# sharinka0715/semantic-gaussians

Hardware: NVIDIA H100
Metric: Mviews/s + HBM GB/s, 1M Gaussians, 256-ch features, 1080p, fwd+bwd (higher is better)
Workload: dtype f32

## Files before the change

semantic-gaussians_b200/csrc/chn_dfeature.cu:

```cuda
#include <cstddef>
#include <cstring>
#include "chn_blend.cuh"
#include "tma.cuh"

namespace sgb {

namespace {

constexpr int kDfCH = 256;
constexpr int kDfStages = 4;
constexpr int kDfPass = 128;
constexpr int kDfSlabPix = 32;
constexpr int kDfSlabs = SGB_TILE_PIX / kDfSlabPix;
constexpr int kDfComputeWarps = kDfCH / 32;
constexpr int kDfThreads = 128 + 32 * kDfComputeWarps;
constexpr uint32_t kDfProducerRegs = 56, kDfComputeRegs = 224;
static_assert(128 * kDfProducerRegs + 32 * kDfComputeWarps * kDfComputeRegs <= 65536,
              "dL/dfeature: the warp groups' register limits exceed the register file");

struct DfHdr {
    int end;
    int cnt;
    int slab;
    int ch0, nch;
    uint32_t gid[kDfPass];
};
template <typename T>
struct DfSmem {
    float w[kDfStages][kDfPass * kDfSlabPix];
    T dl[kDfStages][kDfSlabPix * kDfCH];
    DfHdr hdr[kDfStages];
    uint64_t full[kDfStages], empty[kDfStages];
};
template <typename T>
constexpr size_t kDfSmemBytes = sizeof(DfSmem<T>) + 1024;
static_assert(kDfSmemBytes<float> <= 227 * 1024, "dL/dfeature shared memory exceeds the sm_90 opt-in limit");

__device__ __forceinline__ void df_setmaxnreg_dec() {
    asm volatile("setmaxnreg.dec.sync.aligned.u32 %0;" ::"n"(kDfProducerRegs));
}
__device__ __forceinline__ void df_setmaxnreg_inc() {
    asm volatile("setmaxnreg.inc.sync.aligned.u32 %0;" ::"n"(kDfComputeRegs));
}

template <typename T>
__device__ __forceinline__ int df_swz(int cl) { return sizeof(T) == 4 ? (cl >> 1) & 3 : (cl >> 2) & 1; }
__device__ __forceinline__ float4 df_dl4(const float* dl, int q, int k, int swz, int rs) {
    return *reinterpret_cast<const float4*>(dl + (q >> 2) * rs + k * 16 + (((q & 3) ^ swz ^ (k >> 1)) << 2));
}
__device__ __forceinline__ float4 df_dl4(const __half* dl, int q, int k, int swz, int rs) {
    const uint2 r = *reinterpret_cast<const uint2*>(dl + (q >> 2) * rs + k * 16 + ((((q & 3) >> 1) ^ swz) << 3) +
                                                    ((q & 1) << 2));
    const float2 a = __half22float2(*reinterpret_cast<const __half2*>(&r.x));
    const float2 b = __half22float2(*reinterpret_cast<const __half2*>(&r.y));
    return make_float4(a.x, a.y, b.x, b.y);
}

__device__ __forceinline__ void cp_async4(void* dst_smem, const void* src, int src_bytes) {
    asm volatile("cp.async.ca.shared.global [%0], [%1], 4, %2;" ::"r"(smem_u32(dst_smem)), "l"(src), "r"(src_bytes)
                 : "memory");
}
__device__ __forceinline__ void cp_async_mbar_arrive_noinc(uint64_t* bar) {
    asm volatile("cp.async.mbarrier.arrive.noinc.shared::cta.b64 [%0];" ::"r"(smem_u32(bar)) : "memory");
}

template <int R, typename T>
__device__ __forceinline__ void df_slab(float (&acc)[8][16], const float* __restrict__ ws, const T* __restrict__ dl,
                                        int rs, int eg, int swz) {
#pragma unroll 1
    for (int q = 0; q < kDfSlabPix / 4; q++) {
        float4 d[16];
#pragma unroll
        for (int k = 0; k < 16; k++) d[k] = df_dl4(dl + (k >> 2) * (8 * 16), q, k & 3, swz, rs);
#pragma unroll
        for (int j = 0; j < R; j++) {
            const float4 wv = *reinterpret_cast<const float4*>(ws + (eg + 16 * j) * 32 + ((q ^ (eg & 7)) << 2));
#pragma unroll
            for (int k = 0; k < 16; k++) {
                acc[j][k] = fmaf(wv.x, d[k].x, acc[j][k]);
                acc[j][k] = fmaf(wv.y, d[k].y, acc[j][k]);
                acc[j][k] = fmaf(wv.z, d[k].z, acc[j][k]);
                acc[j][k] = fmaf(wv.w, d[k].w, acc[j][k]);
            }
        }
    }
}

template <typename T>
__global__ void __launch_bounds__(kDfThreads, 1) dfeature_persistent_kernel(
    int W, int H, int C, int CW, const T* __restrict__ dL_dpixels, PoolView pool, float* __restrict__ dL_dcolors,
    int* __restrict__ work_counter, const __grid_constant__ CUtensorMap dl_map,
    const __grid_constant__ CUtensorMap w_map, const int use_tma) {
    extern __shared__ __align__(128) unsigned char smem_raw[];
    DfSmem<T>& sm = *reinterpret_cast<DfSmem<T>*>(smem_raw + ((1024u - (smem_u32(smem_raw) & 1023u)) & 1023u));
    const int tid = threadIdx.x, lane = tid & 31, warp = tid >> 5;
    if (tid == 0) {
        for (int i = 0; i < kDfStages; i++) {
            mbar_init(&sm.full[i], use_tma ? 1 : 33);
            mbar_init(&sm.empty[i], kDfComputeWarps);
        }
        mbar_fence_init();
    }
    __syncthreads();

    if (warp >= 4) {
        df_setmaxnreg_inc();
        const int cw = warp - 4;
        const int eg = lane >> 1;
        const int cl = cw * 32 + (lane & 1) * 4;
        const int rs = CW * 16;
        const int swz = df_swz<T>(cl);
        const bool red16 = ((C & 3) == 0) && ((reinterpret_cast<uintptr_t>(dL_dcolors) & 15) == 0);
        float acc[8][16];
        for (uint32_t step = 0;; step++) {
            const int st = (int)(step % kDfStages);
            mbar_wait(&sm.full[st], (step / kDfStages) & 1u);
            const DfHdr& h = sm.hdr[st];
            if (h.end) break;
            const int slab = h.slab, cnt = h.cnt, nch = h.nch;
            const int R = (cnt + 15) >> 4;
            if (slab == 0) {
#pragma unroll
                for (int j = 0; j < 8; j++)
#pragma unroll
                    for (int k = 0; k < 16; k++) acc[j][k] = 0.f;
            }
            if (cw * 32 < nch) {
                const float* ws = sm.w[st];
                const T* dl = sm.dl[st] + cl * 16;
                switch (R) {
                    case 1: df_slab<1, T>(acc, ws, dl, rs, eg, swz); break;
                    case 2: df_slab<2, T>(acc, ws, dl, rs, eg, swz); break;
                    case 3: df_slab<3, T>(acc, ws, dl, rs, eg, swz); break;
                    case 4: df_slab<4, T>(acc, ws, dl, rs, eg, swz); break;
                    case 5: df_slab<5, T>(acc, ws, dl, rs, eg, swz); break;
                    case 6: df_slab<6, T>(acc, ws, dl, rs, eg, swz); break;
                    case 7: df_slab<7, T>(acc, ws, dl, rs, eg, swz); break;
                    default: df_slab<8, T>(acc, ws, dl, rs, eg, swz); break;
                }
                if (slab == kDfSlabs - 1) {
                    const int ch0 = h.ch0;
#pragma unroll
                    for (int j = 0; j < 8; j++) {
                        const int e = eg + 16 * j;
                        if (j >= R || e >= cnt) continue;
                        float* dst = dL_dcolors + (size_t)h.gid[e] * C + ch0 + cl;
#pragma unroll
                        for (int g = 0; g < 4; g++) {
                            const int c = cl + 8 * g;
                            if (red16 && c + 4 <= nch) {
                                red_add_v4_f32(dst + 8 * g, make_float4(acc[j][4 * g], acc[j][4 * g + 1],
                                                                        acc[j][4 * g + 2], acc[j][4 * g + 3]));
                            } else {
#pragma unroll
                                for (int k = 0; k < 4; k++)
                                    if (c + k < nch) red_add_f32(dst + 8 * g + k, acc[j][4 * g + k]);
                            }
                        }
                    }
                }
            }
            __syncwarp();
            if (lane == 0) mbar_arrive(&sm.empty[st]);
        }
        return;
    }

    df_setmaxnreg_dec();
    if (warp != 0) return;
    const int tiles_x = (W + SGB_TILE - 1) / SGB_TILE;
    const int tiles = tiles_x * ((H + SGB_TILE - 1) / SGB_TILE);
    const int nitems = (C + CW - 1) / CW;
    const int total = tiles * nitems;
    const size_t plane = (size_t)H * W;
    const uint32_t dl_bytes = use_tma ? (uint32_t)(kDfSlabPix * CW * sizeof(T)) : 0u;
    uint32_t step = 0;
    auto acquire = [&]() -> int {
        const int st = (int)(step % kDfStages);
        if (step >= kDfStages) mbar_wait(&sm.empty[st], ((step / kDfStages) - 1) & 1u);
        return st;
    };
    for (;;) {
        int k = 0;
        if (lane == 0) k = atomicAdd(work_counter, 1);
        k = __shfl_sync(0xffffffffu, k, 0);
        if (k >= total) break;
        const int tile = k / nitems, ch0 = (k % nitems) * CW;
        const uint32_t n = pool.count[tile];
        if (n == 0) continue;
        const uint32_t dbase = pool.dirbase[tile];
        const int nch = min(CW, C - ch0);
        const int x0 = (tile % tiles_x) * SGB_TILE, y0 = (tile / tiles_x) * SGB_TILE;
        for (uint32_t base = 0; base < n; base += kDfPass) {
            const int cnt = (int)min((uint32_t)kDfPass, n - base);
            const int nck = (cnt + kChunkEntries - 1) / kChunkEntries;
            const uint32_t cid = lane < nck ? chunk_of(pool, dbase, (int)(base / kChunkEntries) + lane) : 0u;
            uint32_t gid[kDfPass / 32];
#pragma unroll
            for (int i = 0; i < kDfPass / 32; i++) {
                const int e = lane + 32 * i;
                const uint32_t c = __shfl_sync(0xffffffffu, cid, e / kChunkEntries);
                gid[i] = e < cnt ? pool.chunks[c].meta[e & (kChunkEntries - 1)].x : 0u;
            }
            for (int s = 0; s < kDfSlabs; s++) {
                const int st = acquire();
                DfHdr& h = sm.hdr[st];
                if (lane == 0) {
                    h.end = 0;
                    h.cnt = cnt;
                    h.slab = s;
                    h.ch0 = ch0;
                    h.nch = nch;
                }
                if (s == kDfSlabs - 1) {
#pragma unroll
                    for (int i = 0; i < kDfPass / 32; i++) h.gid[lane + 32 * i] = gid[i];
// ... 118 lines not shown
```

semantic-gaussians_b200/csrc/chn_forward.cu:

```cuda
#include "chn_blend.cuh"
#include "tma.cuh"

namespace sgb {

namespace {

template <int MCH>
__device__ __forceinline__ bool acc_nonfinite(const float2 (&acc)[8][MCH / 2]) {
    float2 z = make_float2(0.f, 0.f);
#pragma unroll
    for (int i = 0; i < 8; i++)
#pragma unroll
        for (int k = 0; k < MCH / 2; k++) z = ffma2(acc[i][k], make_float2(0.f, 0.f), z);
    const float t = z.x + z.y;
    return __any_sync(0xffffffffu, t != t);
}

template <int MCH, bool RING>
__device__ __noinline__ void forward_redo_guarded(const PoolView& pool, uint32_t n, uint32_t dbase,
                                                  const float* __restrict__ features, int C, int ch0, int nch,
                                                  int warp, int woff, int cg, const float* __restrict__ bg_color,
                                                  const float* __restrict__ final_T, int W, int H, uint32_t row,
                                                  uint32_t col0, float* __restrict__ out_color) {
    float acc[8][MCH];
#pragma unroll
    for (int i = 0; i < 8; i++)
#pragma unroll
        for (int k = 0; k < MCH; k++) acc[i][k] = 0.f;
    for (uint32_t e = 0; e < n; e++) {
        const WChunk* ck = pool.chunks + chunk_of(pool, dbase, (int)(e / kChunkEntries));
        const int s = (int)(e & (kChunkEntries - 1));
        const uint2 meta = ck->meta[s];
        if (!((meta.y >> warp) & 1u)) continue;
        const float* fr = features + (size_t)meta.x * C + ch0;
        float f[MCH];
#pragma unroll
        for (int k = 0; k < MCH; k++) {
            const int chl = RING ? ((k >> 2) * 32 + cg * 4 + (k & 3)) : (cg * MCH + k);
            f[k] = chl < nch ? __ldg(fr + chl) : 0.f;
        }
#pragma unroll
        for (int i = 0; i < 8; i++) {
            const float w = ck->w[s][woff + i];
            if (w != 0.f) {
#pragma unroll
                for (int k = 0; k < MCH; k++) acc[i][k] = fmaf(f[k], w, acc[i][k]);
            }
        }
    }
    if (row >= (uint32_t)H) return;
    const size_t plane = (size_t)H * W;
#pragma unroll
    for (int k = 0; k < MCH; k++) {
        const int chl = RING ? ((k >> 2) * 32 + cg * 4 + (k & 3)) : (cg * MCH + k);
        if (chl >= nch) continue;
        const float bgc = bg_color[ch0 + chl];
        float* dst = out_color + (size_t)(ch0 + chl) * plane + (size_t)W * row + col0;
#pragma unroll
        for (int i = 0; i < 8; i++)
            if (col0 + i < (uint32_t)W) dst[i] = acc[i][k] + final_T[(size_t)W * row + col0 + i] * bgc;
    }
}

template <int CH>
__global__ void __launch_bounds__(kTileThreads, 2) blend_forward_ldg_kernel(
    int W, int H, int C, const float* __restrict__ features, const float* __restrict__ bg_color,
    const float* __restrict__ final_T, PoolView pool, float* __restrict__ out_color) {
    constexpr int MCH = CH / 8;
    const int tiles_x = (W + SGB_TILE - 1) / SGB_TILE;
    const int nchunksC = (C + CH - 1) / CH;
    const int tile = blockIdx.x / nchunksC;
    const int ch0 = (blockIdx.x % nchunksC) * CH;
    const int nch = min(CH, C - ch0);
    const int tid = threadIdx.x, lane = tid & 31, warp = tid >> 5;
    const int pg = lane >> 3, cg = lane & 7;
    const uint2 pix_min = {(uint32_t)(tile % tiles_x) * SGB_TILE, (uint32_t)(tile / tiles_x) * SGB_TILE};

    float2 acc[8][MCH / 2];
#pragma unroll
    for (int i = 0; i < 8; i++)
#pragma unroll
        for (int k = 0; k < MCH / 2; k++) acc[i][k] = make_float2(0.f, 0.f);

    const uint32_t n = pool.count[tile];
    const uint32_t dbase = pool.dirbase[tile];
    const int woff = warp * 32 + pg * 8;
    const int foff = ch0 + cg * MCH;
    for (uint32_t e = 0; e < n;) {
        const WChunk* ck = pool.chunks + chunk_of(pool, dbase, (int)(e / kChunkEntries));
        const int m = (int)min((uint32_t)kChunkEntries, n - e);
        for (int s = 0; s < m; s++) {
            const uint2 meta = ck->meta[s];
            if (!((meta.y >> warp) & 1u)) continue;
            const float4* wp = reinterpret_cast<const float4*>(&ck->w[s][woff]);
            const float4 w0 = wp[0], w1 = wp[1];
            const float* fr = features + (size_t)meta.x * C + foff;
            float2 f[MCH / 2];
#pragma unroll
            for (int k = 0; k < MCH / 2; k++) {
                f[k].x = (cg * MCH + 2 * k < nch) ? __ldg(fr + 2 * k) : 0.f;
                f[k].y = (cg * MCH + 2 * k + 1 < nch) ? __ldg(fr + 2 * k + 1) : 0.f;
            }
            const float wv[8] = {w0.x, w0.y, w0.z, w0.w, w1.x, w1.y, w1.z, w1.w};
#pragma unroll
            for (int i = 0; i < 8; i++) {
                const float2 w2 = make_float2(wv[i], wv[i]);
#pragma unroll
                for (int k = 0; k < MCH / 2; k++) acc[i][k] = ffma2(f[k], w2, acc[i][k]);
            }
        }
        e += m;
    }
    const uint32_t row = pix_min.y + 2 * warp + (pg >> 1);
    const uint32_t col0 = pix_min.x + (pg & 1) * 8;
    if (acc_nonfinite<MCH>(acc)) {
        forward_redo_guarded<MCH, false>(pool, n, dbase, features, C, ch0, nch, warp, woff, cg, bg_color, final_T, W, H,
                                         row, col0, out_color);
        return;
    }
    if (row < (uint32_t)H) {
        const size_t plane = (size_t)H * W;
        const bool vec = ((W & 3) == 0) && (col0 + 8 <= (uint32_t)W);
        float Tv[8];
#pragma unroll
        for (int i = 0; i < 8; i++) Tv[i] = (col0 + i < (uint32_t)W) ? final_T[(size_t)W * row + col0 + i] : 0.f;
#pragma unroll
        for (int k = 0; k < MCH; k++) {
            const int chl = cg * MCH + k;
            if (chl >= nch) continue;
            const float bgc = bg_color[ch0 + chl];
            float* dst = out_color + (size_t)(ch0 + chl) * plane + (size_t)W * row + col0;
            float o[8];
#pragma unroll
            for (int i = 0; i < 8; i++) o[i] = ((k & 1) ? acc[i][k / 2].y : acc[i][k / 2].x) + Tv[i] * bgc;
            if (vec) {
                reinterpret_cast<float4*>(dst)[0] = make_float4(o[0], o[1], o[2], o[3]);
                reinterpret_cast<float4*>(dst)[1] = make_float4(o[4], o[5], o[6], o[7]);
            } else {
#pragma unroll
                for (int i = 0; i < 8; i++)
                    if (col0 + i < (uint32_t)W) dst[i] = o[i];
            }
        }
    }
}

template <int CH, int NS>
__global__ void __launch_bounds__(kTileThreads, 2) blend_forward_tma_kernel(
    int W, int H, int C, const float* __restrict__ features, const float* __restrict__ bg_color,
    const float* __restrict__ final_T, PoolView pool, float* __restrict__ out_color) {
    constexpr int MCH = CH / 8;
    constexpr int ES = kChunkEntries;
    constexpr int LA = NS - 2;
    constexpr int kDirCap = 192;
    struct Stage {
        float w[ES][SGB_TILE_PIX];
        float f[ES][CH];
    };
    extern __shared__ __align__(128) unsigned char smem_raw[];
    Stage* stg = reinterpret_cast<Stage*>(smem_raw);
    __shared__ uint64_t full_bar[NS], empty_bar[NS];
    __shared__ uint32_t Cdir[kDirCap];
    __shared__ __align__(16) float Tsm[SGB_TILE_PIX];
    __shared__ float bgS[CH];

    const int tiles_x = (W + SGB_TILE - 1) / SGB_TILE;
    const int nchunksC = (C + CH - 1) / CH;
    const int tile = blockIdx.x / nchunksC;
    const int ch0 = (blockIdx.x % nchunksC) * CH;
    const int nch = min(CH, C - ch0);
    const int tid = threadIdx.x, lane = tid & 31, warp = tid >> 5;
    const int pg = lane_group4(lane), cg = lane_group8(lane);
    const uint2 pix_min = {(uint32_t)(tile % tiles_x) * SGB_TILE, (uint32_t)(tile / tiles_x) * SGB_TILE};

    const uint32_t n = pool.count[tile];
    const int nb = (int)((n + ES - 1) / ES);
    const uint32_t dbase = pool.dirbase[tile];
    if (tid == 0) {
        for (int i = 0; i < NS; i++) {
            mbar_init(&full_bar[i], 1);
            mbar_init(&empty_bar[i], kTileThreads / 32);
        }
        mbar_fence_init();
    }
    for (int k = tid; k < min(nb, kDirCap); k += kTileThreads) Cdir[k] = chunk_of(pool, dbase, k);
    {
        const uint32_t x = pix_min.x + (tid & (SGB_TILE - 1)), y = pix_min.y + (tid >> 4);
        Tsm[tid] = (x < (uint32_t)W && y < (uint32_t)H) ? final_T[(size_t)W * y + x] : 0.f;
        if (tid < nch) bgS[tid] = bg_color[ch0 + tid];
    }
    if (nch < CH)
        for (int e = tid; e < NS * ES * CH; e += kTileThreads) {
            const int k = e % CH;
            if (k >= nch) stg[e / (ES * CH)].f[(e / CH) % ES][k] = 0.f;
        }
    __syncthreads();

    auto chunk_ptr = [&](int bi) {
        return pool.chunks + (bi < kDirCap ? Cdir[bi] : chunk_of(pool, dbase, bi));
    };
    auto load_meta = [&](int bi) {
        uint2 m = make_uint2(0u, 0u);
        if (bi < nb && lane < min(ES, (int)n - bi * ES)) m = __ldg(&chunk_ptr(bi)->meta[lane]);
        return m;
    };
    auto issue = [&](int bi, uint2 meta) {
        const int st = bi % NS;
        const int cnt = min(ES, (int)n - bi * ES);
        if (bi >= NS) mbar_wait(&empty_bar[st], (uint32_t)(((bi / NS) - 1) & 1));
        if (lane < cnt) {
            const WChunk* ck = chunk_ptr(bi);
            bulk_g2s(&stg[st].w[lane][0], &ck->w[lane][0], SGB_TILE_PIX * 4u, &full_bar[st]);
            bulk_g2s(&stg[st].f[lane][0], features + (size_t)meta.x * C + ch0, (uint32_t)nch * 4u, &full_bar[st]);
        }
        __syncwarp();
        if (lane == 0) mbar_arrive_expect_tx(&full_bar[st], (uint32_t)cnt * (SGB_TILE_PIX * 4u + (uint32_t)nch * 4u));
    };
    uint2 meta_next = make_uint2(0u, 0u);
    int pb = 0;
    if (warp == 0) {
        uint2 m[LA];
#pragma unroll
        for (int i = 0; i < LA; i++) m[i] = load_meta(i);
#pragma unroll
        for (int i = 0; i < LA; i++)
            if (i < nb) issue(i, m[i]);
        pb = min(LA, nb);
        meta_next = load_meta(pb);
    }

    float2 acc[8][MCH / 2];
#pragma unroll
    for (int i = 0; i < 8; i++)
#pragma unroll
        for (int k = 0; k < MCH / 2; k++) acc[i][k] = make_float2(0.f, 0.f);

    const int woff = warp * 32 + pg * 8;
    auto entry = [&](const Stage& sg, int e) {
        const float4 w0 = *reinterpret_cast<const float4*>(&sg.w[e][woff]);
        const float4 w1 = *reinterpret_cast<const float4*>(&sg.w[e][woff + 4]);
        float2 f[MCH / 2];
#pragma unroll
        for (int q = 0; q < MCH / 4; q++) {
            const float4 t = *reinterpret_cast<const float4*>(&sg.f[e][q * 32 + cg * 4]);
            f[2 * q] = make_float2(t.x, t.y);
            f[2 * q + 1] = make_float2(t.z, t.w);
        }
        const float wv[8] = {w0.x, w0.y, w0.z, w0.w, w1.x, w1.y, w1.z, w1.w};
#pragma unroll
        for (int i = 0; i < 8; i++) {
            const float2 w2 = make_float2(wv[i], wv[i]);
#pragma unroll
            for (int k = 0; k < MCH / 2; k++) acc[i][k] = ffma2(f[k], w2, acc[i][k]);
        }
    };
    for (int b = 0; b < nb; b++) {
        const int st = b % NS;
        const int cnt = min(ES, (int)n - b * ES);
        if (warp == 0 && pb < nb) {
            issue(pb, meta_next);
            pb++;
            meta_next = load_meta(pb);
        }
        mbar_wait(&full_bar[st], (uint32_t)((b / NS) & 1));
        if (cnt == ES) {
#pragma unroll
            for (int e = 0; e < ES; e++) entry(stg[st], e);
        } else {
            for (int e = 0; e < cnt; e++) entry(stg[st], e);
        }
        __syncwarp();
        if (lane == 0) mbar_arrive(&empty_bar[st]);
    }
    const uint32_t row = pix_min.y + 2 * warp + (pg >> 1);
    const uint32_t col0 = pix_min.x + (pg & 1) * 8;
    if (acc_nonfinite<MCH>(acc)) {
        forward_redo_guarded<MCH, true>(pool, n, dbase, features, C, ch0, nch, warp, woff, cg, bg_color, final_T, W, H,
                                        row, col0, out_color);
        return;
    }
    if (row < (uint32_t)H) {
        const size_t plane = (size_t)H * W;
        const bool vec = ((W & 3) == 0) && (col0 + 8 <= (uint32_t)W);
        const float4 t0 = *reinterpret_cast<const float4*>(&Tsm[(2 * warp + (pg >> 1)) * SGB_TILE + (pg & 1) * 8]);
        const float4 t1 = *reinterpret_cast<const float4*>(&Tsm[(2 * warp + (pg >> 1)) * SGB_TILE + (pg & 1) * 8 + 4]);
        const float Tv[8] = {t0.x, t0.y, t0.z, t0.w, t1.x, t1.y, t1.z, t1.w};
#pragma unroll
        for (int k = 0; k < MCH; k++) {
            const int chl = (k >> 2) * 32 + cg * 4 + (k & 3);
            if (chl >= nch) continue;
            const float bgc = bgS[chl];
            float* dst = out_color + (size_t)(ch0 + chl) * plane + (size_t)W * row + col0;
            float o[8];
#pragma unroll
            for (int i = 0; i < 8; i++) o[i] = ((k & 1) ? acc[i][k / 2].y : acc[i][k / 2].x) + Tv[i] * bgc;
            if (vec) {
                reinterpret_cast<float4*>(dst)[0] = make_float4(o[0], o[1], o[2], o[3]);
                reinterpret_cast<float4*>(dst)[1] = make_float4(o[4], o[5], o[6], o[7]);
            } else {
#pragma unroll
                for (int i = 0; i < 8; i++)
                    if (col0 + i < (uint32_t)W) dst[i] = o[i];
            }
        }
    }
}

}

int chn_forward(sgb_ctx* ctx, const ViewState& w, const PoolView& pv, float* out_color, cudaStream_t s) {
    const sgb_view_inputs& in = w.in;
    const int tiles = num_tiles(in);
    const int chunks = (in.C + 63) / 64;
    const bool vec = (in.C % 4 == 0) && ((reinterpret_cast<uintptr_t>(w.colors) & 15) == 0);
    StageTimer t(ctx, ST_BLEND_FWD, s);
    ctx->launches += 1;
    if (vec) {
        constexpr int NS = 5;
        const size_t smem_f = (size_t)NS * kChunkEntries * (SGB_TILE_PIX + 64) * sizeof(float);
        static DeviceOnce fattr;
        if (fattr.first_use_on_device()) {
            SGB_CUDA(cudaFuncSetAttribute(blend_forward_tma_kernel<64, NS>, cudaFuncAttributeMaxDynamicSharedMemorySize,
                                          (int)smem_f));
        }
        blend_forward_tma_kernel<64, NS><<<tiles * chunks, kTileThreads, smem_f, s>>>(in.W, in.H, in.C, w.colors,
                                                                                  in.background, w.im.final_T, pv,
                                                                                  out_color);
    } else {
        blend_forward_ldg_kernel<64><<<tiles * chunks, kTileThreads, 0, s>>>(in.W, in.H, in.C, w.colors, in.background,
                                                                          w.im.final_T, pv, out_color);
    }
    SGB_LAUNCH_CHECK("blend_forward kernel", in.debug, s);
    return SGB_OK;
}

}
```

semantic-gaussians_b200/csrc/tma.cuh:

```cuda
#pragma once
#include <cstdint>
#include <cuda.h>
#include <cuda_runtime.h>

namespace sgb {

using TensorMapEncodeFn = CUresult (*)(CUtensorMap*, CUtensorMapDataType, cuuint32_t, void*, const cuuint64_t*,
                                       const cuuint64_t*, const cuuint32_t*, const cuuint32_t*, CUtensorMapInterleave,
                                       CUtensorMapSwizzle, CUtensorMapL2promotion, CUtensorMapFloatOOBfill);
inline TensorMapEncodeFn tensor_map_encoder() {
    static const TensorMapEncodeFn encode = [] {
        void* fn = nullptr;
        cudaDriverEntryPointQueryResult q;
        if (cudaGetDriverEntryPoint("cuTensorMapEncodeTiled", &fn, cudaEnableDefault, &q) != cudaSuccess ||
            q != cudaDriverEntryPointSuccess)
            fn = nullptr;
        return (TensorMapEncodeFn)fn;
    }();
    return encode;
}

inline bool encode_tiled_map(CUtensorMap* map, CUtensorMapDataType type, int rank, const void* base,
                             const cuuint64_t* dims, const cuuint64_t* strides, const cuuint32_t* box,
                             CUtensorMapSwizzle swizzle) {
    const TensorMapEncodeFn encode = tensor_map_encoder();
    const cuuint32_t estr[5] = {1, 1, 1, 1, 1};
    return encode &&
           encode(map, type, (cuuint32_t)rank, const_cast<void*>(base), dims, strides, box, estr,
                  CU_TENSOR_MAP_INTERLEAVE_NONE, swizzle, CU_TENSOR_MAP_L2_PROMOTION_L2_128B,
                  CU_TENSOR_MAP_FLOAT_OOB_FILL_NONE) == CUDA_SUCCESS;
}

#ifdef __CUDACC__
__device__ __forceinline__ uint32_t smem_u32(const void* p) {
    return (uint32_t)__cvta_generic_to_shared(p);
}
__device__ __forceinline__ void mbar_init(uint64_t* bar, uint32_t count) {
    asm volatile("mbarrier.init.shared::cta.b64 [%0], %1;" ::"r"(smem_u32(bar)), "r"(count) : "memory");
}
__device__ __forceinline__ void mbar_fence_init() {
    asm volatile("fence.mbarrier_init.release.cluster;" ::: "memory");
}
__device__ __forceinline__ void mbar_arrive_expect_tx(uint64_t* bar, uint32_t bytes) {
    asm volatile("mbarrier.arrive.expect_tx.shared::cta.b64 _, [%0], %1;" ::"r"(smem_u32(bar)), "r"(bytes)
                 : "memory");
}
__device__ __forceinline__ void mbar_arrive(uint64_t* bar) {
    asm volatile("mbarrier.arrive.shared::cta.b64 _, [%0];" ::"r"(smem_u32(bar)) : "memory");
}
__device__ __forceinline__ void mbar_wait(uint64_t* bar, uint32_t parity) {
    uint32_t done = 0;
    for (uint32_t spins = 0; !done; spins++) {
        asm volatile(
            "{\n\t.reg .pred p;\n\t"
            "mbarrier.try_wait.parity.shared::cta.b64 p, [%1], %2;\n\t"
            "selp.u32 %0, 1, 0, p;\n\t}"
            : "=r"(done)
            : "r"(smem_u32(bar)), "r"(parity)
            : "memory");
        if (spins > (1u << 24)) __trap();
    }
}
__device__ __forceinline__ void bulk_g2s(void* dst_smem, const void* src_gmem, uint32_t bytes, uint64_t* bar) {
    asm volatile("cp.async.bulk.shared::cluster.global.mbarrier::complete_tx::bytes [%0], [%1], %2, [%3];" ::"r"(
                     smem_u32(dst_smem)),
                 "l"(src_gmem), "r"(bytes), "r"(smem_u32(bar))
                 : "memory");
}
__device__ __forceinline__ void tma_tile2d_g2s(void* dst_smem, const CUtensorMap* map, int x, int y, uint64_t* bar) {
    asm volatile(
        "cp.async.bulk.tensor.2d.shared::cluster.global.tile.mbarrier::complete_tx::bytes [%0], [%1, {%2, %3}], [%4];" ::"r"(
            smem_u32(dst_smem)),
        "l"(reinterpret_cast<uint64_t>(map)), "r"(x), "r"(y), "r"(smem_u32(bar))
        : "memory");
}
__device__ __forceinline__ void tma_tile3d_g2s(void* dst_smem, const CUtensorMap* map, int x, int y, int z, uint64_t* bar) {
    asm volatile(
        "cp.async.bulk.tensor.3d.shared::cluster.global.tile.mbarrier::complete_tx::bytes [%0], [%1, {%2, %3, %4}], [%5];" ::"r"(
            smem_u32(dst_smem)),
        "l"(reinterpret_cast<uint64_t>(map)), "r"(x), "r"(y), "r"(z), "r"(smem_u32(bar))
        : "memory");
}
__device__ __forceinline__ void fence_proxy_async_smem() { asm volatile("fence.proxy.async.shared::cta;" ::: "memory"); }
#endif

}
```

Before: 0.00007157.

## Rewrite forward blend as persistent warp-specialized kernel with TMA output stores

Replaces the per-tile/per-channel-chunk forward blend kernels with a persistent kernel. A producer warp pulls work items from an atomic counter and stages weight and feature chunks into a 4-stage mbarrier ring, while compute warps with raised register budgets accumulate 128-channel slices. Results go out through a 3D TMA store from shared memory. The aim is to remove launch and tail overhead, improve overlap of loads with FMAs, and widen channel slices from 64 to 128 so the weight data is reused more. In exchange it needs large shared memory, runs one block per SM, and adds more complex synchronization.

```diff
diff --git a/semantic-gaussians_b200/csrc/chn_dfeature.cu b/semantic-gaussians_b200/csrc/chn_dfeature.cu
--- a/semantic-gaussians_b200/csrc/chn_dfeature.cu
+++ b/semantic-gaussians_b200/csrc/chn_dfeature.cu
@@ -54,14 +54,6 @@
     const float2 a = __half22float2(*reinterpret_cast<const __half2*>(&r.x));
     const float2 b = __half22float2(*reinterpret_cast<const __half2*>(&r.y));
     return make_float4(a.x, a.y, b.x, b.y);
-}
-
-__device__ __forceinline__ void cp_async4(void* dst_smem, const void* src, int src_bytes) {
-    asm volatile("cp.async.ca.shared.global [%0], [%1], 4, %2;" ::"r"(smem_u32(dst_smem)), "l"(src), "r"(src_bytes)
-                 : "memory");
-}
-__device__ __forceinline__ void cp_async_mbar_arrive_noinc(uint64_t* bar) {
-    asm volatile("cp.async.mbarrier.arrive.noinc.shared::cta.b64 [%0];" ::"r"(smem_u32(bar)) : "memory");
 }
 
 template <int R, typename T>
diff --git a/semantic-gaussians_b200/csrc/chn_forward.cu b/semantic-gaussians_b200/csrc/chn_forward.cu
--- a/semantic-gaussians_b200/csrc/chn_forward.cu
+++ b/semantic-gaussians_b200/csrc/chn_forward.cu
@@ -1,3 +1,4 @@
+#include <cstring>
 #include "chn_blend.cuh"
 #include "tma.cuh"
 
@@ -5,38 +6,74 @@
 
 namespace {
 
-template <int MCH>
-__device__ __forceinline__ bool acc_nonfinite(const float2 (&acc)[8][MCH / 2]) {
-    float2 z = make_float2(0.f, 0.f);
+constexpr int kFwCH = 128;
+constexpr int kFwStages = 4;
+constexpr int kFwComputeWarps = SGB_TILE_PIX / 32;
+constexpr int kFwThreads = 128 + 32 * kFwComputeWarps;
+constexpr uint32_t kFwProducerRegs = 56, kFwComputeRegs = 224;
+static_assert(128 * kFwProducerRegs + 32 * kFwComputeWarps * kFwComputeRegs <= 65536,
+              "forward: the warp groups' register limits exceed the register file");
+
+struct FwHdr {
+    int end;
+    int cnt;
+    int first, last;
+    int tile, ch0, nch;
+    uint32_t n, dbase;
+};
+struct FwStage {
+    float w[kChunkEntries][SGB_TILE_PIX];
+    float f[kChunkEntries][kFwCH];
+};
+struct FwSmem {
+    FwStage stg[kFwStages];
+    float out[kFwComputeWarps][kFwCH][2][SGB_TILE];
+    FwHdr hdr[kFwStages];
+    uint64_t full[kFwStages], empty[kFwStages];
+};
+constexpr size_t kFwSmemBytes = sizeof(FwSmem);
+static_assert(kFwSmemBytes <= 227 * 1024, "forward shared memory exceeds the sm_90 opt-in limit");
+
+__device__ __forceinline__ void fw_setmaxnreg_dec() {
+    asm volatile("setmaxnreg.dec.sync.aligned.u32 %0;" ::"n"(kFwProducerRegs));
+}
+__device__ __forceinline__ void fw_setmaxnreg_inc() {
+    asm volatile("setmaxnreg.inc.sync.aligned.u32 %0;" ::"n"(kFwComputeRegs));
+}
+
+__device__ __forceinline__ int fw_channel(int k, int cg) { return (k >> 2) * 32 + cg * 4 + (k & 3); }
+
+__device__ __forceinline__ bool acc_nonfinite(const float (&acc)[8][16]) {
+    float z0 = 0.f, z1 = 0.f;
 #pragma unroll
     for (int i = 0; i < 8; i++)
 #pragma unroll
-        for (int k = 0; k < MCH / 2; k++) z = ffma2(acc[i][k], make_float2(0.f, 0.f), z);
-    const float t = z.x + z.y;
+        for (int k = 0; k < 16; k += 2) {
+            z0 = fmaf(acc[i][k], 0.f, z0);
+            z1 = fmaf(acc[i][k + 1], 0.f, z1);
+        }
+    const float t = z0 + z1;
     return __any_sync(0xffffffffu, t != t);
 }
 
-template <int MCH, bool RING>
-__device__ __noinline__ void forward_redo_guarded(const PoolView& pool, uint32_t n, uint32_t dbase,
-                                                  const float* __restrict__ features, int C, int ch0, int nch,
-                                                  int warp, int woff, int cg, const float* __restrict__ bg_color,
-                                                  const float* __restrict__ final_T, int W, int H, uint32_t row,
-                                                  uint32_t col0, float* __restrict__ out_color) {
-    float acc[8][MCH];
+__device__ __forceinline__ void forward_redo_guarded(float (&acc)[8][16], const PoolView& pool, uint32_t n,
+                                                     uint32_t dbase, const float* __restrict__ features, int C,
+                                                     int ch0, int nch, int strip, int woff, int cg) {
 #pragma unroll
     for (int i = 0; i < 8; i++)
 #pragma unroll
-        for (int k = 0; k < MCH; k++) acc[i][k] = 0.f;
+        for (int k = 0; k < 16; k++) acc[i][k] = 0.f;
+#pragma unroll 1
     for (uint32_t e = 0; e < n; e++) {
         const WChunk* ck = pool.chunks + chunk_of(pool, dbase, (int)(e / kChunkEntries));
         const int s = (int)(e & (kChunkEntries - 1));
         const uint2 meta = ck->meta[s];
-        if (!((meta.y >> warp) & 1u)) continue;
+        if (!((meta.y >> strip) & 1u)) continue;
         const float* fr = features + (size_t)meta.x * C + ch0;
-        float f[MCH];
-#pragma unroll
-        for (int k = 0; k < MCH; k++) {
-            const int chl = RING ? ((k >> 2) * 32 + cg * 4 + (k & 3)) : (cg * MCH + k);
+        float f[16];
+#pragma unroll
+        for (int k = 0; k < 16; k++) {
+            const int chl = fw_channel(k, cg);
             f[k] = chl < nch ? __ldg(fr + chl) : 0.f;
         }
 #pragma unroll
@@ -44,293 +81,289 @@
             const float w = ck->w[s][woff + i];
             if (w != 0.f) {
 #pragma unroll
-                for (int k = 0; k < MCH; k++) acc[i][k] = fmaf(f[k], w, acc[i][k]);
-            }
-        }
-    }
-    if (row >= (uint32_t)H) return;
-    const size_t plane = (size_t)H * W;
-#pragma unroll
-    for (int k = 0; k < MCH; k++) {
-        const int chl = RING ? ((k >> 2) * 32 + cg * 4 + (k & 3)) : (cg * MCH + k);
-        if (chl >= nch) continue;
-        const float bgc = bg_color[ch0 + chl];
-        float* dst = out_color + (size_t)(ch0 + chl) * plane + (size_t)W * row + col0;
-#pragma unroll
-        for (int i = 0; i < 8; i++)
-            if (col0 + i < (uint32_t)W) dst[i] = acc[i][k] + final_T[(size_t)W * row + col0 + i] * bgc;
-    }
-}
-
-template <int CH>
-__global__ void __launch_bounds__(kTileThreads, 2) blend_forward_ldg_kernel(
-    int W, int H, int C, const float* __restrict__ features, const float* __restrict__ bg_color,
-    const float* __restrict__ final_T, PoolView pool, float* __restrict__ out_color) {
-    constexpr int MCH = CH / 8;
+                for (int k = 0; k < 16; k++) acc[i][k] = fmaf(f[k], w, acc[i][k]);
+            }
+        }
+    }
+}
+
+template <int NQ, bool MASK>
+__device__ __forceinline__ void fw_entry(float (&acc)[8][16], const float* __restrict__ wr,
+                                         const float* __restrict__ fr, bool last_ok) {
+    const float4 w0 = *reinterpret_cast<const float4*>(wr);
+    const float4 w1 = *reinterpret_cast<const float4*>(wr + 4);
+    float4 f[NQ];
+#pragma unroll
+    for (int q = 0; q < NQ; q++) f[q] = *reinterpret_cast<const float4*>(fr + q * 32);
+    if (MASK && !last_ok) f[NQ - 1] = make_float4(0.f, 0.f, 0.f, 0.f);
+    const float wv[8] = {w0.x, w0.y, w0.z, w0.w, w1.x, w1.y, w1.z, w1.w};
+#pragma unroll
+    for (int i = 0; i < 8; i++) {
+#pragma unroll
+        for (int q = 0; q < NQ; q++) {
+            acc[i][4 * q + 0] = fmaf(f[q].x, wv[i], acc[i][4 * q + 0]);
+            acc[i][4 * q + 1] = fmaf(f[q].y, wv[i], acc[i][4 * q + 1]);
+            acc[i][4 * q + 2] = fmaf(f[q].z, wv[i], acc[i][4 * q + 2]);
+            acc[i][4 * q + 3] = fmaf(f[q].w, wv[i], acc[i][4 * q + 3]);
+        }
+    }
+}
+
+template <int NQ, bool MASK>
+__device__ __forceinline__ void fw_chunk(float (&acc)[8][16], const float* __restrict__ ws,
+                                         const float* __restrict__ fs, int cnt, bool last_ok) {
+    if (cnt == kChunkEntries) {
+#pragma unroll
+        for (int e = 0; e < kChunkEntries; e++)
+            fw_entry<NQ, MASK>(acc, ws + e * SGB_TILE_PIX, fs + e * kFwCH, last_ok);
+    } else {
+#pragma unroll 1
+        for (int e = 0; e < cnt; e++) fw_entry<NQ, MASK>(acc, ws + e * SGB_TILE_PIX, fs + e * kFwCH, last_ok);
+    }
+}
+
+__global__ void __launch_bounds__(kFwThreads, 1) blend_forward_persistent_kernel(
+    int W, int H, int C, int CW, const float* __restrict__ features, const float* __restrict__ bg_color,
+    const float* __restrict__ final_T, PoolView pool, float* __restrict__ out_color, int* __restrict__ work_counter,
+    const int use_bulk, const __grid_constant__ CUtensorMap out_map, const int use_tma_store) {
+    extern __shared__ __align__(128) unsigned char smem_raw[];
+    FwSmem& sm = *reinterpret_cast<FwSmem*>(smem_raw);
+    const int tid = threadIdx.x, lane = tid & 31, warp = tid >> 5;
     const int tiles_x = (W + SGB_TILE - 1) / SGB_TILE;
-    const int nchunksC = (C + CH - 1) / CH;
-    const int tile = blockIdx.x / nchunksC;
-    const int ch0 = (blockIdx.x % nchunksC) * CH;
-    const int nch = min(CH, C - ch0);
-    const int tid = threadIdx.x, lane = tid & 31, warp = tid >> 5;
-    const int pg = lane >> 3, cg = lane & 7;
-    const uint2 pix_min = {(uint32_t)(tile % tiles_x) * SGB_TILE, (uint32_t)(tile / tiles_x) * SGB_TILE};
-
-    float2 acc[8][MCH / 2];
-#pragma unroll
-    for (int i = 0; i < 8; i++)
-#pragma unroll
-        for (int k = 0; k < MCH / 2; k++) acc[i][k] = make_float2(0.f, 0.f);
-
-    const uint32_t n = pool.count[tile];
-    const uint32_t dbase = pool.dirbase[tile];
-    const int woff = warp * 32 + pg * 8;
-    const int foff = ch0 + cg * MCH;
-    for (uint32_t e = 0; e < n;) {
-        const WChunk* ck = pool.chunks + chunk_of(pool, dbase, (int)(e / kChunkEntries));
-        const int m = (int)min((uint32_t)kChunkEntries, n - e);
-        for (int s = 0; s < m; s++) {
-            const uint2 meta = ck->meta[s];
-            if (!((meta.y >> warp) & 1u)) continue;
-            const float4* wp = reinterpret_cast<const float4*>(&ck->w[s][woff]);
-            const float4 w0 = wp[0], w1 = wp[1];
-            const float* fr = features + (size_t)meta.x * C + foff;
-            float2 f[MCH / 2];
-#pragma unroll
-            for (int k = 0; k < MCH / 2; k++) {
-                f[k].x = (cg * MCH + 2 * k < nch) ? __ldg(fr + 2 * k) : 0.f;
-                f[k].y = (cg * MCH + 2 * k + 1 < nch) ? __ldg(fr + 2 * k + 1) : 0.f;
-            }
-            const float wv[8] = {w0.x, w0.y, w0.z, w0.w, w1.x, w1.y, w1.z, w1.w};
-#pragma unroll
-            for (int i = 0; i < 8; i++) {
-                const float2 w2 = make_float2(wv[i], wv[i]);
-#pragma unroll
-                for (int k = 0; k < MCH / 2; k++) acc[i][k] = ffma2(f[k], w2, acc[i][k]);
-            }
-        }
-        e += m;
-    }
-    const uint32_t row = pix_min.y + 2 * warp + (pg >> 1);
-    const uint32_t col0 = pix_min.x + (pg & 1) * 8;
-    if (acc_nonfinite<MCH>(acc)) {
-        forward_redo_guarded<MCH, false>(pool, n, dbase, features, C, ch0, nch, warp, woff, cg, bg_color, final_T, W, H,
-                                         row, col0, out_color);
+    if (tid == 0) {
+        for (int i = 0; i < kFwStages; i++) {
+            mbar_init(&sm.full[i], use_bulk ? 1 : 33);
+            mbar_init(&sm.empty[i], kFwComputeWarps);
+        }
+        mbar_fence_init();
+    }
+    __syncthreads();
+
+    if (warp >= 4) {
+        fw_setmaxnreg_inc();
+        const int strip = warp - 4;
+        const int pg = lane_group4(lane), cg = lane_group8(lane);
+        const int woff = strip * 32 + pg * 8;
+        const size_t plane = (size_t)H * W;
+        float acc[8][16];
+        float Tl = 0.f, bgl[4] = {0.f, 0.f, 0.f, 0.f};
+        for (uint32_t step = 0;; step++) {
+            const int st = (int)(step % kFwStages);
+            mbar_wait(&sm.full[st], (step / kFwStages) & 1u);
+            const FwHdr& h = sm.hdr[st];
+            if (h.end) break;
+            const int cnt = h.cnt, last = h.last, tile = h.tile, ch0 = h.ch0, nch = h.nch;
+            const uint32_t n = h.n, dbase = h.dbase;
+            const uint32_t x0 = (uint32_t)(tile % tiles_x) * SGB_TILE, y0 = (uint32_t)(tile / tiles_x) * SGB_TILE;
+            if (h.first) {
+#pragma unroll
+                for (int i = 0; i < 8; i++)
+#pragma unroll
+                    for (int k = 0; k < 16; k++) acc[i][k] = 0.f;
+                const uint32_t x = x0 + (lane & 15), y = y0 + 2 * strip + (lane >> 4);
+                Tl = (x < (uint32_t)W && y < (uint32_t)H) ? __ldg(final_T + (size_t)W * y + x) : 0.f;
+#pragma unroll
+                for (int q = 0; q < 4; q++) bgl[q] = lane + 32 * q < nch ? __ldg(bg_color + ch0 + lane + 32 * q) : 0.f;
+            }
+            if (cnt > 0) {
+                const float* ws = &sm.stg[st].w[0][woff];
+                const float* fs = &sm.stg[st].f[0][cg * 4];
+                const int nq = (nch + 31) >> 5;
+                const bool last_ok = (nq - 1) * 32 + cg * 4 < nch;
+                if (nq == 4 && (nch & 31) == 0) {
+                    fw_chunk<4, false>(acc, ws, fs, cnt, true);
+                } else {
+                    switch (nq) {
+                        case 1: fw_chunk<1, true>(acc, ws, fs, cnt, last_ok); break;
+                        case 2: fw_chunk<2, true>(acc, ws, fs, cnt, last_ok); break;
+                        case 3: fw_chunk<3, true>(acc, ws, fs, cnt, last_ok); break;
+                        default: fw_chunk<4, true>(acc, ws, fs, cnt, last_ok); break;
+                    }
+                }
+            }
+            __syncwarp();
+            if (lane == 0) mbar_arrive(&sm.empty[st]);
+            if (!last) continue;
+
+            const uint32_t row = y0 + 2 * strip + (pg >> 1);
+            const uint32_t col0 = x0 + (pg & 1) * 8;
+            float Tv[8], bgv[16];
+#pragma unroll
+            for (int i = 0; i < 8; i++) Tv[i] = __shfl_sync(0xffffffffu, Tl, pg * 8 + i);
+#pragma unroll
+            for (int k = 0; k < 16; k++) bgv[k] = __shfl_sync(0xffffffffu, bgl[k >> 2], cg * 4 + (k & 3));
+            if (acc_nonfinite(acc)) forward_redo_guarded(acc, pool, n, dbase, features, C, ch0, nch, strip, woff, cg);
+            if (use_tma_store) {
+                float(&box)[kFwCH][2][SGB_TILE] = sm.out[strip];
+                if (lane == 0) bulk_wait_read_all();
+                __syncwarp();
+#pragma unroll
+                for (int k = 0; k < 16; k++) {
+                    float o[8];
+#pragma unroll
+                    for (int i = 0; i < 8; i++) o[i] = acc[i][k] + Tv[i] * bgv[k];
+                    float4* dst = reinterpret_cast<float4*>(&box[fw_channel(k, cg)][pg >> 1][(pg & 1) * 8]);
+                    dst[0] = make_float4(o[0], o[1], o[2], o[3]);
+                    dst[1] = make_float4(o[4], o[5], o[6], o[7]);
+                }
+                fence_proxy_async_smem();
+                __syncwarp();
+                if (lane == 0) tma_store3d_s2g(&out_map, (int)x0, (int)y0 + 2 * strip, ch0, &box[0][0][0]);
+            } else if (row < (uint32_t)H) {
+                const bool vec = ((W & 3) == 0) && (col0 + 8 <= (uint32_t)W);
+#pragma unroll
+                for (int k = 0; k < 16; k++) {
+                    const int chl = fw_channel(k, cg);
+                    if (chl >= nch) continue;
+                    float* dst = out_color + (size_t)(ch0 + chl) * plane + (size_t)W * row + col0;
+                    float o[8];
+#pragma unroll
+                    for (int i = 0; i < 8; i++) o[i] = acc[i][k] + Tv[i] * bgv[k];
+                    if (vec) {
+                        reinterpret_cast<float4*>(dst)[0] = make_float4(o[0], o[1], o[2], o[3]);
+                        reinterpret_cast<float4*>(dst)[1] = make_float4(o[4], o[5], o[6], o[7]);
+                    } else {
+#pragma unroll
+                        for (int i = 0; i < 8; i++)
+                            if (col0 + i < (uint32_t)W) dst[i] = o[i];
+                    }
+                }
+            }
+        }
+        if (use_tma_store && lane == 0) bulk_wait_all();
         return;
     }
-    if (row < (uint32_t)H) {
-        const size_t plane = (size_t)H * W;
-        const bool vec = ((W & 3) == 0) && (col0 + 8 <= (uint32_t)W);
-        float Tv[8];
-#pragma unroll
-        for (int i = 0; i < 8; i++) Tv[i] = (col0 + i < (uint32_t)W) ? final_T[(size_t)W * row + col0 + i] : 0.f;
-#pragma unroll
-        for (int k = 0; k < MCH; k++) {
-            const int chl = cg * MCH + k;
-            if (chl >= nch) continue;
-            const float bgc = bg_color[ch0 + chl];
-            float* dst = out_color + (size_t)(ch0 + chl) * plane + (size_t)W * row + col0;
-            float o[8];
-#pragma unroll
-            for (int i = 0; i < 8; i++) o[i] = ((k & 1) ? acc[i][k / 2].y : acc[i][k / 2].x) + Tv[i] * bgc;
-            if (vec) {
-                reinterpret_cast<float4*>(dst)[0] = make_float4(o[0], o[1], o[2], o[3]);
-                reinterpret_cast<float4*>(dst)[1] = make_float4(o[4], o[5], o[6], o[7]);
+
+    fw_setmaxnreg_dec();
+    if (warp != 0) return;
+    const int tiles = tiles_x * ((H + SGB_TILE - 1) / SGB_TILE);
+    const int nitems = (C + CW - 1) / CW;
+    const int total = tiles * nitems;
+    uint32_t step = 0;
+    auto acquire = [&]() -> int {
+        const int st = (int)(step % kFwStages);
+        if (step >= kFwStages) mbar_wait(&sm.empty[st], ((step / kFwStages) - 1) & 1u);
+        return st;
+    };
+    for (;;) {
+        int k = 0;
+        if (lane == 0) k = atomicAdd(work_counter, 1);
+        k = __shfl_sync(0xffffffffu, k, 0);
+        if (k >= total) break;
+        const int tile = k / nitems, ch0 = (k % nitems) * CW;
+        const int nch = min(CW, C - ch0);
+        const int nch4 = (nch + 3) & ~3;
+        const uint32_t n = pool.count[tile];
+        const uint32_t dbase = pool.dirbase[tile];
+        const int nck = (int)((n + kChunkEntries - 1) / kChunkEntries);
+        uint32_t cid = 0u;
+        auto chunk_id = [&](int j) {
+            if ((j & 31) == 0) cid = lane < nck - j ? chunk_of(pool, dbase, j + lane) : 0u;
+            return __shfl_sync(0xffffffffu, cid, j & 31);
+        };
+        auto gid_of = [&](uint32_t c, int j) {
+            const int cntj = min(kChunkEntries, (int)n - j * kChunkEntries);
+            return lane < cntj ? __ldg(&pool.chunks[c].meta[lane].x) : 0u;
+        };
+        uint32_t c_cur = 0u, g_cur = 0u;
+        if (nck > 0) {
+            c_cur = chunk_id(0);
+            g_cur = gid_of(c_cur, 0);
+        }
+        for (int j = 0; j < max(nck, 1); j++) {
+            const int cnt = nck > 0 ? min(kChunkEntries, (int)n - j * kChunkEntries) : 0;
+            uint32_t c_next = 0u, g_next = 0u;
+            if (j + 1 < nck) {
+                c_next = chunk_id(j + 1);
+                g_next = gid_of(c_next, j + 1);
+            }
+            const int st = acquire();
+            FwHdr& h = sm.hdr[st];
+            if (lane == 0) {
+                h.end = 0;
+                h.cnt = cnt;
+                h.first = j == 0;
+                h.last = j + 1 >= nck;
+                h.tile = tile;
+                h.ch0 = ch0;
+                h.nch = nch;
+                h.n = n;
+                h.dbase = dbase;
+            }
+            FwStage& sg = sm.stg[st];
+            if (cnt > 0 && lane == 0)
+                bulk_g2s(&sg.w[0][0], &pool.chunks[c_cur].w[0][0], (uint32_t)cnt * (SGB_TILE_PIX * 4u), &sm.full[st]);
+            if (use_bulk) {
+                if (lane < cnt)
+                    bulk_g2s(&sg.f[lane][0], features + (size_t)g_cur * C + ch0, (uint32_t)nch * 4u, &sm.full[st]);
             } else {
-#pragma unroll
-                for (int i = 0; i < 8; i++)
-                    if (col0 + i < (uint32_t)W) dst[i] = o[i];
-            }
-        }
-    }
-}
-
-template <int CH, int NS>
-__global__ void __launch_bounds__(kTileThreads, 2) blend_forward_tma_kernel(
-    int W, int H, int C, const float* __restrict__ features, const float* __restrict__ bg_color,
-    const float* __restrict__ final_T, PoolView pool, float* __restrict__ out_color) {
-    constexpr int MCH = CH / 8;
-    constexpr int ES = kChunkEntries;
-    constexpr int LA = NS - 2;
-    constexpr int kDirCap = 192;
-    struct Stage {
-        float w[ES][SGB_TILE_PIX];
-        float f[ES][CH];
-    };
-    extern __shared__ __align__(128) unsigned char smem_raw[];
-    Stage* stg = reinterpret_cast<Stage*>(smem_raw);
-    __shared__ uint64_t full_bar[NS], empty_bar[NS];
-    __shared__ uint32_t Cdir[kDirCap];
-    __shared__ __align__(16) float Tsm[SGB_TILE_PIX];
-    __shared__ float bgS[CH];
-
-    const int tiles_x = (W + SGB_TILE - 1) / SGB_TILE;
-    const int nchunksC = (C + CH - 1) / CH;
-    const int tile = blockIdx.x / nchunksC;
-    const int ch0 = (blockIdx.x % nchunksC) * CH;
-    const int nch = min(CH, C - ch0);
-    const int tid = threadIdx.x, lane = tid & 31, warp = tid >> 5;
-    const int pg = lane_group4(lane), cg = lane_group8(lane);
-    const uint2 pix_min = {(uint32_t)(tile % tiles_x) * SGB_TILE, (uint32_t)(tile / tiles_x) * SGB_TILE};
-
-    const uint32_t n = pool.count[tile];
-    const int nb = (int)((n + ES - 1) / ES);
-    const uint32_t dbase = pool.dirbase[tile];
-    if (tid == 0) {
-        for (int i = 0; i < NS; i++) {
-            mbar_init(&full_bar[i], 1);
-            mbar_init(&empty_bar[i], kTileThreads / 32);
-        }
-        mbar_fence_init();
-    }
-    for (int k = tid; k < min(nb, kDirCap); k += kTileThreads) Cdir[k] = chunk_of(pool, dbase, k);
-    {
-        const uint32_t x = pix_min.x + (tid & (SGB_TILE - 1)), y = pix_min.y + (tid >> 4);
-        Tsm[tid] = (x < (uint32_t)W && y < (uint32_t)H) ? final_T[(size_t)W * y + x] : 0.f;
-        if (tid < nch) bgS[tid] = bg_color[ch0 + tid];
-    }
-    if (nch < CH)
-        for (int e = tid; e < NS * ES * CH; e += kTileThreads) {
-            const int k = e % CH;
-            if (k >= nch) stg[e / (ES * CH)].f[(e / CH) % ES][k] = 0.f;
-        }
-    __syncthreads();
-
-    auto chunk_ptr = [&](int bi) {
-        return pool.chunks + (bi < kDirCap ? Cdir[bi] : chunk_of(pool, dbase, bi));
-    };
-    auto load_meta = [&](int bi) {
-        uint2 m = make_uint2(0u, 0u);
-        if (bi < nb && lane < min(ES, (int)n - bi * ES)) m = __ldg(&chunk_ptr(bi)->meta[lane]);
-        return m;
-    };
-    auto issue = [&](int bi, uint2 meta) {
-        const int st = bi % NS;
-        const int cnt = min(ES, (int)n - bi * ES);
-        if (bi >= NS) mbar_wait(&empty_bar[st], (uint32_t)(((bi / NS) - 1) & 1));
-        if (lane < cnt) {
-            const WChunk* ck = chunk_ptr(bi);
-            bulk_g2s(&stg[st].w[lane][0], &ck->w[lane][0], SGB_TILE_PIX * 4u, &full_bar[st]);
-            bulk_g2s(&stg[st].f[lane][0], features + (size_t)meta.x * C + ch0, (uint32_t)nch * 4u, &full_bar[st]);
-        }
-        __syncwarp();
-        if (lane == 0) mbar_arrive_expect_tx(&full_bar[st], (uint32_t)cnt * (SGB_TILE_PIX * 4u + (uint32_t)nch * 4u));
-    };
-    uint2 meta_next = make_uint2(0u, 0u);
-    int pb = 0;
-    if (warp == 0) {
-        uint2 m[LA];
-#pragma unroll
-        for (int i = 0; i < LA; i++) m[i] = load_meta(i);
-#pragma unroll
-        for (int i = 0; i < LA; i++)
-            if (i < nb) issue(i, m[i]);
-        pb = min(LA, nb);
-        meta_next = load_meta(pb);
-    }
-
-    float2 acc[8][MCH / 2];
-#pragma unroll
-    for (int i = 0; i < 8; i++)
-#pragma unroll
-        for (int k = 0; k < MCH / 2; k++) acc[i][k] = make_float2(0.f, 0.f);
-
-    const int woff = warp * 32 + pg * 8;
-    auto entry = [&](const Stage& sg, int e) {
-        const float4 w0 = *reinterpret_cast<const float4*>(&sg.w[e][woff]);
-        const float4 w1 = *reinterpret_cast<const float4*>(&sg.w[e][woff + 4]);
-        float2 f[MCH / 2];
-#pragma unroll
-        for (int q = 0; q < MCH / 4; q++) {
-            const float4 t = *reinterpret_cast<const float4*>(&sg.f[e][q * 32 + cg * 4]);
-            f[2 * q] = make_float2(t.x, t.y);
-            f[2 * q + 1] = make_float2(t.z, t.w);
-        }
-        const float wv[8] = {w0.x, w0.y, w0.z, w0.w, w1.x, w1.y, w1.z, w1.w};
-#pragma unroll
-        for (int i = 0; i < 8; i++) {
-            const float2 w2 = make_float2(wv[i], wv[i]);
-#pragma unroll
-            for (int k = 0; k < MCH / 2; k++) acc[i][k] = ffma2(f[k], w2, acc[i][k]);
-        }
-    };
-    for (int b = 0; b < nb; b++) {
-        const int st = b % NS;
-        const int cnt = min(ES, (int)n - b * ES);
-        if (warp == 0 && pb < nb) {
-            issue(pb, meta_next);
-            pb++;
-            meta_next = load_meta(pb);
-        }
-        mbar_wait(&full_bar[st], (uint32_t)((b / NS) & 1));
-        if (cnt == ES) {
-#pragma unroll
-            for (int e = 0; e < ES; e++) entry(stg[st], e);
-        } else {
-            for (int e = 0; e < cnt; e++) entry(stg[st], e);
-        }
-        __syncwarp();
-        if (lane == 0) mbar_arrive(&empty_bar[st]);
-    }
-    const uint32_t row = pix_min.y + 2 * warp + (pg >> 1);
-    const uint32_t col0 = pix_min.x + (pg & 1) * 8;
-    if (acc_nonfinite<MCH>(acc)) {
-        forward_redo_guarded<MCH, true>(pool, n, dbase, features, C, ch0, nch, warp, woff, cg, bg_color, final_T, W, H,
-                                        row, col0, out_color);
-        return;
-    }
-    if (row < (uint32_t)H) {
-        const size_t plane = (size_t)H * W;
-        const bool vec = ((W & 3) == 0) && (col0 + 8 <= (uint32_t)W);
-        const float4 t0 = *reinterpret_cast<const float4*>(&Tsm[(2 * warp + (pg >> 1)) * SGB_TILE + (pg & 1) * 8]);
-        const float4 t1 = *reinterpret_cast<const float4*>(&Tsm[(2 * warp + (pg >> 1)) * SGB_TILE + (pg & 1) * 8 + 4]);
-        const float Tv[8] = {t0.x, t0.y, t0.z, t0.w, t1.x, t1.y, t1.z, t1.w};
-#pragma unroll
-        for (int k = 0; k < MCH; k++) {
-            const int chl = (k >> 2) * 32 + cg * 4 + (k & 3);
-            if (chl >= nch) continue;
-            const float bgc = bgS[chl];
-            float* dst = out_color + (size_t)(ch0 + chl) * plane + (size_t)W * row + col0;
-            float o[8];
-#pragma unroll
-            for (int i = 0; i < 8; i++) o[i] = ((k & 1) ? acc[i][k / 2].y : acc[i][k / 2].x) + Tv[i] * bgc;
-            if (vec) {
-                reinterpret_cast<float4*>(dst)[0] = make_float4(o[0], o[1], o[2], o[3]);
-                reinterpret_cast<float4*>(dst)[1] = make_float4(o[4], o[5], o[6], o[7]);
-            } else {
-#pragma unroll
-                for (int i = 0; i < 8; i++)
-                    if (col0 + i < (uint32_t)W) dst[i] = o[i];
-            }
-        }
-    }
-}
-
+#pragma unroll 1
+                for (int e = 0; e < cnt; e++) {
+                    const float* src = features + (size_t)__shfl_sync(0xffffffffu, g_cur, e) * C + ch0;
+                    for (int c = lane; c < nch4; c += 32) cp_async4(&sg.f[e][c], c < nch ? src + c : src, c < nch ? 4 : 0);
+                }
+                cp_async_mbar_arrive_noinc(&sm.full[st]);
+            }
+            __syncwarp();
+            if (lane == 0)
+                mbar_arrive_expect_tx(&sm.full[st], (uint32_t)cnt * (SGB_TILE_PIX * 4u + (use_bulk ? (uint32_t)nch * 4u : 0u)));
+            step++;
+            c_cur = c_next;
+            g_cur = g_next;
+        }
+    }
+    const int st = acquire();
+    if (lane == 0) sm.hdr[st].end = 1;
+    __syncwarp();
+    if (!use_bulk) mbar_arrive(&sm.full[st]);
+    if (lane == 0) mbar_arrive(&sm.full[st]);
+}
+
+}
+
+static bool encode_forward_out_map(CUtensorMap* map, float* out, int W, int H, int C, int CW) {
+    memset(map, 0, sizeof(*map));
+    if ((W & 3) != 0 || (reinterpret_cast<uintptr_t>(out) & 15) != 0) return false;
+    const cuuint64_t dims[3] = {(cuuint64_t)W, (cuuint64_t)H, (cuuint64_t)C};
+    const cuuint64_t strides[2] = {(cuuint64_t)W * sizeof(float), (cuuint64_t)W * H * sizeof(float)};
+    const cuuint32_t box[3] = {SGB_TILE, 2, (cuuint32_t)CW};
+    return encode_tiled_map(map, CU_TENSOR_MAP_DATA_TYPE_FLOAT32, 3, out, dims, strides, box,
+                            CU_TENSOR_MAP_SWIZZLE_NONE);
 }
 
 int chn_forward(sgb_ctx* ctx, const ViewState& w, const PoolView& pv, float* out_color, cudaStream_t s) {
     const sgb_view_inputs& in = w.in;
-    const int tiles = num_tiles(in);
-    const int chunks = (in.C + 63) / 64;
-    const bool vec = (in.C % 4 == 0) && ((reinterpret_cast<uintptr_t>(w.colors) & 15) == 0);
+    const int nitems = (in.C + kFwCH - 1) / kFwCH;
+    const int CW = ((in.C + nitems - 1) / nitems + 15) / 16 * 16;
+    const int items = num_tiles(in) * nitems;
+    if (items == 0) return SGB_OK;
+    const int use_bulk = (in.C % 4 == 0) && ((reinterpret_cast<uintptr_t>(w.colors) & 15) == 0);
+    CUtensorMap out_map;
+    const int use_tma_store = encode_forward_out_map(&out_map, out_color, in.W, in.H, in.C, CW) ? 1 : 0;
+    int rc = ctx->work.ensure(sizeof(int));
+    if (rc) return rc;
+    static DeviceOnce attr_set;
+    static int grid_of_device[64];
+    int dev = 0;
+    SGB_CUDA(cudaGetDevice(&dev));
+    int& grid = grid_of_device[dev < 64 ? dev : 63];
+    if (attr_set.first_use_on_device()) {
+        SGB_CUDA(cudaFuncSetAttribute(blend_forward_persistent_kernel, cudaFuncAttributeMaxDynamicSharedMemorySize,
+                                      (int)kFwSmemBytes));
+        int per_sm = 0, sms = 0;
+        SGB_CUDA(cudaOccupancyMaxActiveBlocksPerMultiprocessor(&per_sm, blend_forward_persistent_kernel, kFwThreads,
+                                                               kFwSmemBytes));
+        SGB_CUDA(cudaDeviceGetAttribute(&sms, cudaDevAttrMultiProcessorCount, dev));
+        grid = per_sm * sms > 0 ? per_sm * sms : 1;
+    }
+    int* counter = static_cast<int*>(ctx->work.p);
     StageTimer t(ctx, ST_BLEND_FWD, s);
+    SGB_CUDA(cudaMemsetAsync(counter, 0, sizeof(int), s));
     ctx->launches += 1;
-    if (vec) {
-        constexpr int NS = 5;
-        const size_t smem_f = (size_t)NS * kChunkEntries * (SGB_TILE_PIX + 64) * sizeof(float);
-        static DeviceOnce fattr;
-        if (fattr.first_use_on_device()) {
-            SGB_CUDA(cudaFuncSetAttribute(blend_forward_tma_kernel<64, NS>, cudaFuncAttributeMaxDynamicSharedMemorySize,
-                                          (int)smem_f));
-        }
-        blend_forward_tma_kernel<64, NS><<<tiles * chunks, kTileThreads, smem_f, s>>>(in.W, in.H, in.C, w.colors,
-                                                                                  in.background, w.im.final_T, pv,
-                                                                                  out_color);
-    } else {
-        blend_forward_ldg_kernel<64><<<tiles * chunks, kTileThreads, 0, s>>>(in.W, in.H, in.C, w.colors, in.background,
-                                                                          w.im.final_T, pv, out_color);
-    }
-    SGB_LAUNCH_CHECK("blend_forward kernel", in.debug, s);
+    blend_forward_persistent_kernel<<<grid < items ? grid : items, kFwThreads, kFwSmemBytes, s>>>(
+        in.W, in.H, in.C, CW, w.colors, in.background, w.im.final_T, pv, out_color, counter, use_bulk, out_map,
+        use_tma_store);
+    SGB_LAUNCH_CHECK("blend_forward_persistent_kernel", in.debug, s);
     return SGB_OK;
 }
 
diff --git a/semantic-gaussians_b200/csrc/tma.cuh b/semantic-gaussians_b200/csrc/tma.cuh
--- a/semantic-gaussians_b200/csrc/tma.cuh
+++ b/semantic-gaussians_b200/csrc/tma.cuh
@@ -81,6 +81,22 @@
         "l"(reinterpret_cast<uint64_t>(map)), "r"(x), "r"(y), "r"(z), "r"(smem_u32(bar))
         : "memory");
 }
+__device__ __forceinline__ void tma_store3d_s2g(const CUtensorMap* map, int x, int y, int z, const void* src_smem) {
+    asm volatile("cp.async.bulk.tensor.3d.global.shared::cta.bulk_group [%0, {%1, %2, %3}], [%4];" ::"l"(
+                     reinterpret_cast<uint64_t>(map)),
+                 "r"(x), "r"(y), "r"(z), "r"(smem_u32(src_smem))
+                 : "memory");
+    asm volatile("cp.async.bulk.commit_group;" ::: "memory");
+}
+__device__ __forceinline__ void bulk_wait_read_all() { asm volatile("cp.async.bulk.wait_group.read 0;" ::: "memory"); }
+__device__ __forceinline__ void bulk_wait_all() { asm volatile("cp.async.bulk.wait_group 0;" ::: "memory"); }
+__device__ __forceinline__ void cp_async4(void* dst_smem, const void* src, int src_bytes) {
+    asm volatile("cp.async.ca.shared.global [%0], [%1], 4, %2;" ::"r"(smem_u32(dst_smem)), "l"(src), "r"(src_bytes)
+                 : "memory");
+}
+__device__ __forceinline__ void cp_async_mbar_arrive_noinc(uint64_t* bar) {
+    asm volatile("cp.async.mbarrier.arrive.noinc.shared::cta.b64 [%0];" ::"r"(smem_u32(bar)) : "memory");
+}
 __device__ __forceinline__ void fence_proxy_async_smem() { asm volatile("fence.proxy.async.shared::cta;" ::: "memory"); }
 #endif
 
```

After: 0.00007467, median of 6. 4.3% higher.
